# itmo153277/JoshUpscale

Hardware: AMD Instinct MI355X
Metric: frames/sec 480x270->1920x1080 recurrent SR (higher is better)
Workload: dtype bf16

## Files before the change

### joshupscale_amd/csrc/dev_switch.cpp

```cpp
#include "dev_switch.h"

#ifdef JU_TEST_HOOKS
#include <cstdlib>
#endif

namespace ju {

#ifdef JU_TEST_HOOKS
const char *devSwitch(Dev which) {
	static const char *const kNames[static_cast<int>(Dev::Count)] = {
	    "JU_TAIL", "JU_PACK", "JU_POOL", "JU_UPSAMPLE", "JU_FLOW_CONV", "JU_TOWER", "JU_CALIBRATE", "JU_FLOW", "JU_DIRECT",
	    "JU_DIRECT_GRAPH", "JU_SYNC_SPIN_US", "JU_TRACE_STEPS", "JU_TRACE_NOSYNC", "JU_RES_BLOCK", "JU_FLOW_TILE",
	    "JU_FLOW_WIDE", "JU_WAVE_PRIO", "JU_CONV_DBUF", "JU_TOWER_FAST", "JU_FP8_GRID", "JU_FP8_BLOCK",
	};
	const int i = static_cast<int>(which);
	if (i < 0 || i >= static_cast<int>(Dev::Count)) return nullptr;
	return std::getenv(kNames[i]);
}
#else
const char *devSwitch(Dev) {
	return nullptr;
}
#endif

}
```

### joshupscale_amd/csrc/dev_switch.h

```cpp
#pragma once

namespace ju {

enum class Dev : int {
	Tail,
	Pack,
	Pool,
	Upsample,
	FlowConv,
	Tower,
	Calibrate,
	Flow,
	Direct,
	DirectGraph,
	SyncSpinUs,
	TraceSteps,
	TraceNoSync,
	ResBlock,
	FlowTile,
	FlowWide,
	WavePrio,
	ConvDbuf,
	TowerFast,
	Fp8Grid,
	Fp8Block,
	Count
};

const char *devSwitch(Dev which);

}
```

### joshupscale_amd/csrc/engine.cpp

```cpp
#include "engine.h"

#include <cstdio>

#include <algorithm>
#include <atomic>
#include <cstdlib>
#include <cstring>
#include <memory>
#include <mutex>
#include <sstream>
#include <stdexcept>

#include "dev_switch.h"
#include "fp8.h"
#include "graphics.h"
#include "log.h"

namespace ju {

namespace {
thread_local int g_DryLaunches = 0;
}
bool launchesAreDry() { return g_DryLaunches > 0; }
DryLaunchScope::DryLaunchScope() { ++g_DryLaunches; }
// ... 284 lines not shown
	const int PH = c.paddedHeight(), PW = c.paddedWidth();
	const int padTop = (PH - H) / 2, padLeft = (PW - W) / 2;
	const FrameIO *io = &m_IO;
	const FrameIO *batchIO = m_BatchIO;
	const void *const *groupPrev = m_GroupPrev;
	void *const *groupOut = m_GroupOut;
	const void *packedIn = m_Packed[set].get();
	void *packedOut = m_Packed[set ^ 1].get();
	const int nIn = c.numFlowInputs;
	const unsigned *sums = c.normalizeBrightness ? m_TailB2.as<unsigned>() + 4 : nullptr;
	auto T = [&](const std::string &n) -> void * { return (batch ? m_BatchTensors : m_Tensors).at(n).buf.get(); };
	auto Op = [&](const std::string &n) { return batch ? Operand{T(n), 0} : operand(n); };
	auto itemBytes = [&](const std::string &n) -> long {
		const Tensor &t = m_Tensors.at(n);
		return static_cast<long>(t.count) * (t.isF32 ? 4 : 2);
	};
	auto noBatch = [&](const char *what) {
		if (batch) throw std::logic_error(std::string("look-ahead: no batched form of ") + what);
	};
	const Operand none{};
	const bool packInBlock = flowPacksInBlock();
	if (batch && (!packInBlock || sums != nullptr)) noBatch("the input packing");
	Operand cur{packedOut, 0};
	long curItem = 0;
	int h = PH, w = PW;
	bool flowHeadDone = false;
	const int nb = static_cast<int>(c.flowFilters.size()) / 2;
	auto fusesUpsample = [&](const std::string &next, int cin) {
		auto it = m_Convs.find(next);
		return m_FusedUpsample && it != m_Convs.end() && cin % 64 == 0 && it->second.nb == 1 &&
		       it->second.cout <= 32;
	};
	const int flowAct = c.flowActivation == 1 ? 2 : 1;
	auto addBlockStep = [&](const std::string &convA, const std::string &convB, const void *in, long inItem,
	                        const std::string &outName, int bh, int bw, bool ups, bool pool, bool outHead, int act2) {
		const ConvWeights &wa = m_Convs.at(convA), &wb = m_Convs.at(convB);
		FlowBlockLaunch fb{};
		fb.in = in;
		fb.w1 = wa.w.get();
		fb.b1 = wa.bias.as<float>();
		fb.w2 = wb.w.get();
		fb.b2 = wb.bias.as<float>();
		fb.out = T(outName);
		fb.H = bh;
		fb.W = bw;
		fb.cin = wa.cinP;
		fb.cmid = wa.cout;
		fb.upsample = ups;
		fb.pool = pool;
		fb.outHead = outHead;
		fb.act1 = flowAct;
		fb.act2 = act2;
		fb.slope = c.flowNegativeSlope;
		fb.items = items;
		fb.inItemBytes = inItem;
		fb.outItemBytes = itemBytes(outName);
		const double flops =
		    items * 2.0 * bh * bw * 9.0 * (double(wa.cinReal) * wa.cout + double(wb.cinReal) * wb.cout);
		if (packInBlock && convA == "flow/block_1/conv_1") {
			fb.packPrev = packedIn;
			fb.packOut = packedOut;
			fb.frameH = H;
			fb.frameW = W;
			fb.padTop = padTop;
			fb.padLeft = padLeft;
			fb.numInputs = nIn;
			fb.sums = sums;
			if (group) {
				fb.packPrev = nullptr;
				fb.packOut = nullptr;
				fb.independentItems = true;
			}
			prog.push_back({"flow", flops, [dt, fb, io, batchIO, groupPrev, groupOut, items, group](hipStream_t s) {
				                FlowBlockLaunch f = fb;
				                f.packFrame = io->in;
				                f.packFrameStride = io->inStride;
				                for (int i = 0; i < items && (items > 1 || group); ++i) {
					                f.packFrames[i] = batchIO[i].in;
					                f.packFrameStrides[i] = batchIO[i].inStride;
					                if (group) {
						                f.packPrevs[i] = groupPrev[i];
						                f.packOuts[i] = groupOut[i];
					                }
				                }
				                launchFlowBlock(dt, f, s);
			                }});
			return;
		}
		prog.push_back({"flow", flops, [dt, fb](hipStream_t s) { launchFlowBlock(dt, fb, s); }});
	};
	auto unitUpsIn = [&](int k) { return k < static_cast<int>(m_FlowUnits.size()) && m_FlowUnits[k].fused && m_FlowUnits[k].upsIn; };
	bool upsampleNext = false;
	for (int i = 0; i < 2 * nb; ++i) {
		const std::string n = "flow/block_" + std::to_string(i + 1);
		const int f = c.flowFilters[i];
		if (m_FlowUnits[i].fused) {
			const bool pool = i < nb;
			if (upsampleNext != m_FlowUnits[i].upsIn) throw std::logic_error("flow plan out of step");
			addBlockStep(n + "/conv_1", n + "/conv_2", cur.ptr, curItem, pool ? n + "/resample" : n + "/a_2", h, w,
			    upsampleNext, pool, false, flowAct);
			upsampleNext = false;
			if (pool) {
				h /= 2;
				w /= 2;
				cur = Operand{T(n + "/resample"), 0};
				curItem = itemBytes(n + "/resample");
// ... 100 lines not shown
	const FrameIO *io = &m_IO;
	const void *packedIn = m_Packed[set].get();
	void *packedOut = m_Packed[set ^ 1].get();
	m_StateBind[set].in = m_State[c.recurrent() ? set : 0].get();
	m_StateBind[set].out = m_State[c.recurrent() ? set ^ 1 : 0].get();
	const StateBind *sb = &m_StateBind[set];
	const int nIn = c.numFlowInputs;
	auto T = [&](const std::string &n) -> void * { return m_Tensors.at(n).buf.get(); };
	auto Op = [&](const std::string &n) { return operand(n); };
	const Operand none{};

	const unsigned *sums = c.normalizeBrightness && c.recurrent() ? m_TailB2.as<unsigned>() + 4 : nullptr;
	std::uint8_t *const discard = c.outputsPreWarp() ? m_DiscardFrame.as<std::uint8_t>() : nullptr;
	const std::ptrdiff_t discardStride = static_cast<std::ptrdiff_t>(W) * 16;
	auto genOutU8 = [=] { return discard ? discard : io->out; };
	auto genOutStride = [=] { return discard ? discardStride : io->outStride; };
	if (!c.recurrent()) {
		const Operand genInOp = Op("gen_in");
		void *genIn = genInOp.ptr;
		const int genPitch = genInOp.pitch;
		prog.push_back({"lr_pack", 0.0,
		    [=](hipStream_t s) { launchLrPack(dt, io->in, io->inStride, genIn, genPitch, H, W, s); }});
	}
	if (sums) {
		unsigned *sumsOut = m_TailB2.as<unsigned>() + 4;
		prog.push_back({"pack", 0.0,
		    [=](hipStream_t s) { launchFrameSums(io->in, io->inStride, H, W, sumsOut, s); }});
	}
	const bool packInBlock = flowPacksInBlock();
	if (!packInBlock && c.recurrent()) {
		prog.push_back({"pack", 0.0, [=](hipStream_t s) {
			                launchPackFrames(dt, io->in, io->inStride, packedIn, packedOut, H, W, PH, PW,
			                    padTop, padLeft, nIn, sums, s);
		                }});
	}
	auto addResBlockStep = [&](const std::string &tag, const std::string &block, Operand in, Operand out,
	                           int bh, int bw, int act, float slope) {
		const ConvWeights &wa = m_Convs.at(block + "/conv_1"), &wb = m_Convs.at(block + "/conv_2");
		FlowBlockLaunch fb{};
		fb.in = in.ptr;
		fb.inPitch = in.pitch;
		fb.w1 = wa.wBlock.get();
		fb.b1 = wa.bias.as<float>();
		fb.w2 = wb.wBlock.get();
		fb.b2 = wb.bias.as<float>();
		fb.out = out.ptr;
		fb.outPitch = out.pitch;
		fb.H = bh;
		fb.W = bw;
		fb.cin = fb.cmid = 64;
		fb.residual = true;
		fb.act1 = fb.act2 = act;
		fb.slope = slope;
		prog.push_back({tag, 2.0 * bh * bw * 9.0 * 64 * 64 * 2,
		    [dt, fb](hipStream_t s) { launchFlowBlock(dt, fb, s); }});
	};
	Operand cur{packedOut, 0};
	int h = PH, w = PW;
	bool flowHeadDone = false;
	if (!c.recurrent()) {
		flowHeadDone = true;
	} else if (c.flowArch == 0) {
		addFlowAutoencoder(&prog, set, 1);
		flowHeadDone = true;
	} else if (m_ResidentFlow) {
		void *in64 = T("flow/in64");
		prog.push_back({"flow", 0.0,
		    [=](hipStream_t s) { launchExpandChannels(dt, packedOut, in64, PH * PW, s); }});
		ResidentTowerParams rp{};
		rp.in = in64;
		rp.inPitch = PW;
		rp.hasHead = 1;
		rp.out = Op("flow/trunk").ptr;
		rp.weights = m_FlowTowerW.get();
		rp.bias = m_FlowTowerB.as<float>();
		rp.mailbox = m_FlowMail.get();
		rp.counters = m_FlowFlags.as<unsigned>();
		rp.error = m_ResErrorDev;
		rp.debug = m_Tensors.at("tower_profile").buf.get();
		rp.H = PH;
		rp.W = PW;
		rp.GX = m_FlowGX;
		rp.GY = m_FlowGY;
		rp.RH = m_FlowRH;
		rp.nLayers = 1 + 2 * c.flowResBlocks;
		rp.leaky = c.flowActivation == 1 ? 1 : 0;
		rp.slope = c.flowNegativeSlope;
		prog.push_back({"flow",
		    2.0 * PH * PW * 9.0 * (3.0 * c.numFlowInputs * 64 + 64.0 * 64 * 2 * c.flowResBlocks),
		    [=](hipStream_t s) { launchResidentTower(dt, rp, s); }});
		cur = Op("flow/trunk");
	} else {
		addConvStep(&prog, "flow", "flow/conv_1", cur, none, Op("flow/x0"), h, w, true, false);
		const char *xs[2] = {"flow/x0", "flow/x1"};
		int a = 0;
		for (int i = 0; i < c.flowResBlocks; ++i) {
			const std::string n = "flow/block_" + std::to_string(i + 1);
			if (m_BlockFused && c.flowResFilters == 64) {
				addResBlockStep("flow", n, Op(xs[a]), Op(xs[a ^ 1]), h, w, c.flowActivation == 1 ? 2 : 1,
				    c.flowNegativeSlope);
				a ^= 1;
				continue;
			}
			addConvStep(&prog, "flow", n + "/conv_1", Op(xs[a]), none, Op("flow/t"), h, w, true, false);
			addConvStep(&prog, "flow", n + "/conv_2", Op("flow/t"), Op(xs[a]), Op(xs[a ^ 1]), h, w,
			    true, false);
// ... 237 lines not shown
			                launchTail(dt, y, w2, b2, io->in, io->inStride, sb->out, genOutU8(),
			                    genOutStride(), H, W, sums, s);
		                }});
	}
	if (c.temporalStrength > 0.0f) {
		const void *preWarp = T("pre_warp");
		unsigned long long *acc = m_TemporalAcc.as<unsigned long long>();
		const TemporalParams tp{c.temporalStrength, c.temporalThreshold, c.temporalGain, c.temporalWindow,
		    c.temporalL2 ? 1 : 0, c.temporalLimit ? 1 : 0, c.temporalLuma ? 1 : 0};
		prog.push_back({"temporal", 0.0, [=](hipStream_t s) {
			                launchTemporalFilter(sb->out, preWarp, genOutU8(), genOutStride(), H, W, sums,
			                    acc, tp, s);
		                }});
	}
}

Engine::Engine(int device, const void *blob, std::size_t size, int dtypeOverride)
    : m_Device(device) {
	int current = -1;
	JU_HIP(hipGetDevice(&current));
	if (current != device) throw std::logic_error("Engine must be created with its device current");
	ModelFile model(blob, size);
	m_Config = model.config();
	const ModelConfig &c = m_Config;
	int dt = dtypeOverride >= 0 ? dtypeOverride : c.computeDtype;
	m_ModelDigest = 14695981039346656037ull;
	for (std::size_t i = 0; i < size; ++i) {
		m_ModelDigest = (m_ModelDigest ^ static_cast<const unsigned char *>(blob)[i]) * 1099511628211ull;
	}
	m_DtypeOverride = dt;
	if (dt == 2) {
		if (c.genFilters != 64 || c.genBlocks < 1) {
			throw std::invalid_argument("fp8 tower needs a 64-filter generator with at least one residual block");
		}
		m_Fp8Tower = true;
		dt = kF16;
	}
	if (dt != kF16 && dt != kBF16) throw std::invalid_argument("Unsupported compute dtype");
	m_DType = static_cast<DType>(dt);
	const int H = c.frameHeight, W = c.frameWidth;
	const int PH = c.paddedHeight(), PW = c.paddedWidth();

	const char *tailMode = devSwitch(Dev::Tail);
	m_FusedTail = !(tailMode && std::string(tailMode) == "split");
	m_TailInTower = !(tailMode && (std::string(tailMode) == "fused" || std::string(tailMode) == "split"));
	const char *packMode = devSwitch(Dev::Pack);
	m_PackInBlock = !(packMode && std::string(packMode) == "split");
	const char *poolMode = devSwitch(Dev::Pool);
	m_FusedPool = !(poolMode && std::string(poolMode) == "split");
	const char *upMode = devSwitch(Dev::Upsample);
	m_FusedUpsample = !(upMode && std::string(upMode) == "split");
	const char *flowConv = devSwitch(Dev::FlowConv);
	m_FlowFused = !(flowConv && std::string(flowConv) == "generic") && m_FusedUpsample;
	planFlowUnits();

	buildWeights(model);

	{
		const char *mode = devSwitch(Dev::Tower);
		int cus = 0;
		JU_HIP(hipDeviceGetAttribute(&cus, hipDeviceAttributeMultiprocessorCount, device));
		bool wanted = !(mode && (std::string(mode) == "layers" || std::string(mode) == "convs"));
		m_BlockFused = !(mode && std::string(mode) == "convs");
		const char *calib = devSwitch(Dev::Calibrate);
		m_Calibrate = calib && calib[0] == '1';
		if (m_Calibrate) {
			if (m_Fp8Tower) throw std::invalid_argument("calibration mode: calibrate the fp16 / bf16 engine, not the 8-bit one");
			wanted = false;
			m_BlockFused = false;
		}
		if (wanted && c.genFilters == 64 && c.genBlocks >= 1 &&
		    residentTowerGeometry(c.frameHeight, c.frameWidth, cus, &m_ResGX, &m_ResGY, &m_ResRH)) {
			m_Resident = m_ResidentCapable = true;
			m_TowerW = DeviceBuffer(m_TowerHostW.size() * 2);
			m_TowerW.upload(m_TowerHostW.data(), m_TowerHostW.size() * 2);
			m_TowerB = DeviceBuffer(m_TowerHostB.size() * 4);
			m_TowerB.upload(m_TowerHostB.data(), m_TowerHostB.size() * 4);
			m_ResMail = DeviceBuffer(m_Fp8Tower ? residentMailboxBytes8(m_ResGX, m_ResGY, c.genActivation == 1)
			                                    : residentMailboxBytes(m_ResGX, m_ResGY, c.genActivation == 1));
			m_ResFlags = DeviceBuffer(residentCounterBytes(m_ResGX, m_ResGY));
			m_ResError = PinnedWords(64);
			m_ResErrorDev = m_ResError.device();
		}
		m_TowerHostW.clear();
		m_TowerHostW.shrink_to_fit();
		const char *flowMode = devSwitch(Dev::Flow);
		if (flowMode && std::string(flowMode) == "convs") m_BlockFused = false;
		if (m_Resident && !(flowMode && (std::string(flowMode) == "layers" || std::string(flowMode) == "convs")) &&
		    c.flowArch == 1 &&
		    c.flowResFilters == 64 && c.flowResBlocks >= 1 && 3 * c.numFlowInputs <= 64 &&
		    residentTowerGeometry(PH, PW, cus, &m_FlowGX, &m_FlowGY, &m_FlowRH)) {
			m_ResidentFlow = m_ResidentFlowCapable = true;
			m_FlowTowerW = DeviceBuffer(m_FlowTowerHostW.size() * 2);
			m_FlowTowerW.upload(m_FlowTowerHostW.data(), m_FlowTowerHostW.size() * 2);
			m_FlowTowerB = DeviceBuffer(m_FlowTowerHostB.size() * 4);
			m_FlowTowerB.upload(m_FlowTowerHostB.data(), m_FlowTowerHostB.size() * 4);
			m_FlowMail = DeviceBuffer(residentMailboxBytes(m_FlowGX, m_FlowGY, c.flowActivation == 1));
			m_FlowFlags = DeviceBuffer(residentCounterBytes(m_FlowGX, m_FlowGY));
		}
		m_FlowTowerHostW.clear();
		m_FlowTowerHostW.shrink_to_fit();
	}

	const std::size_t lr = static_cast<std::size_t>(H) * W;
	const std::size_t plr = static_cast<std::size_t>(PH) * PW;
	m_InStage = DeviceBuffer(lr * 4);
// ... 1698 lines not shown
```

### joshupscale_amd/csrc/engine.h

```cpp
#pragma once

#include <cstddef>
#include <cstdint>
#include <functional>
#include <map>
#include <memory>
#include <mutex>
#include <set>
#include <string>
#include <tuple>
#include <vector>

#include "hip_util.h"
#include "kernels.h"
#include "model.h"

namespace ju {

enum class Location : std::uint8_t { Host = 0, Device = 1, GraphicsResource = 2 };

struct Frame {
	void *ptr;
	Location location;
	std::ptrdiff_t stride;
// ... 120 lines not shown
	void runProgram();
	struct FrameIO {
		const std::uint8_t *in = nullptr;
		std::ptrdiff_t inStride = 0;
		std::uint8_t *out = nullptr;
		std::ptrdiff_t outStride = 0;
	};
	FrameIO m_IO;
	struct StateBind {
		const void *in = nullptr;
		void *out = nullptr;
	};
	StateBind m_StateBind[2];
	const void *m_FlowCur = nullptr;
	bool m_DirectIO = false;
	bool m_PreferDirect = true;
	void submit(const Frame &in, const Frame &out);

	int m_Device;
	ModelConfig m_Config;
	DType m_DType;
	Stream m_Stream;
	bool m_UseGraph = true;
	unsigned m_SpinUs = 2000;
	int m_Idx = 0;
	std::string m_TrunkOut = "trunk_a";

	std::map<std::string, Tensor> m_Tensors;
	std::map<std::string, ConvWeights> m_Convs;
	struct Fp8Conv {
		DeviceBuffer w, scaleA;
	};
	bool m_Fp8Tower = false;
	std::map<std::string, Fp8Conv> m_Fp8Convs;
	std::map<std::string, FoldedConv> m_Fp8Folded;
	DeviceBuffer m_Fp8X, m_Fp8T;
	std::vector<int> m_Fp8Exp;
	DeviceBuffer m_Fp8TowerW, m_Fp8TowerScaleA, m_Fp8TowerBias, m_Fp8TowerScaleB, m_Fp8TowerMul;
	DeviceBuffer m_TailW2, m_TailB2, m_TailW2Frag;
	DeviceBuffer m_Zeros;
	DeviceBuffer m_TemporalAcc;
	struct FlowUnit {
		bool fused = false;
		bool upsIn = false;
	};
	std::vector<FlowUnit> m_FlowUnits;
	bool m_FlowFused = true;
	bool m_BlockFused = true;
	bool m_Calibrate = false;
	void planFlowUnits();
	bool flowConvIsFused(const std::string &name) const;
	bool m_FusedUpsample = true;
	bool m_FusedPool = true;
	bool m_PackInBlock = true;
	bool m_FusedTail = true;
	bool m_TailInTower = false;
	DeviceBuffer m_InStage, m_OutStage, m_RawStage;
	DeviceBuffer m_DiscardFrame;
	DeviceBuffer m_State[2], m_Packed[2];
	bool m_Resident = false;
	int m_ResGX = 0, m_ResGY = 0, m_ResRH = 0;
	std::vector<std::uint16_t> m_TowerHostW;
	std::vector<float> m_TowerHostB;
	DeviceBuffer m_TowerW, m_TowerB, m_ResMail, m_ResFlags;
	bool m_ResidentFlow = false;
	int m_FlowGX = 0, m_FlowGY = 0, m_FlowRH = 0;
	std::vector<std::uint16_t> m_FlowTowerHostW;
	std::vector<float> m_FlowTowerHostB;
	DeviceBuffer m_FlowTowerW, m_FlowTowerB, m_FlowMail, m_FlowFlags;
	bool m_ResidentCapable = false, m_ResidentFlowCapable = false;
	unsigned m_RetryBase = 512, m_RetryAfter = 0, m_CleanFrames = 0, m_Fallbacks = 0;
	void restoreResident();
	void maybeRestoreResident();
	Event m_FrameDone;
	std::unique_lock<std::mutex> chainBegin();
	void chainEnd(std::unique_lock<std::mutex> &lock);
	PinnedWords m_ResError;
	unsigned *m_ResErrorDev = nullptr;
	unsigned takeResidentError();
	void fallbackToLayers(unsigned code);
	std::vector<Step> m_Program[2];
	GraphExec m_Graph[2];
	struct DirectKey {
		const void *in;
		std::ptrdiff_t inStride;
		void *out;
		std::ptrdiff_t outStride;
		int idx;
		bool operator<(const DirectKey &o) const {
			return std::tie(in, inStride, out, outStride, idx) <
			       std::tie(o.in, o.inStride, o.out, o.outStride, o.idx);
		}
	};
	struct DirectEntry {
		GraphExec graph;
		unsigned seen = 0;
		std::uint64_t lastUse = 0;
		bool registered = false;
	};
	std::map<DirectKey, DirectEntry> m_DirectGraphs;
	std::set<DirectKey> m_RegisteredPairs;
	bool directEligible(const Frame &in, const Frame &out) const;
	DirectEntry &directEntry(const DirectKey &key);
	void captureDirect(DirectEntry *e, int idx);
	FrameIO m_BatchIO[kFlowBatchMax];
	struct YuvKey {
// ... 73 lines not shown
```

### joshupscale_amd/csrc/flow_kernels.hip

```cpp
#include "flow_block_common.h"

namespace ju {

namespace {

struct FlowBlockParams {
	const void *in;
	const void *w1;
	const float *b1;
	const void *w2;
	const float *b2;
	void *out;
	int H, W;
	int inPitch, outPitch;
	int act1, act2;
	float slope;
	int skip;
	int prio;
	const void *packPrev;
	void *packOut;
	int frameH, frameW, padTop, padLeft, numInputs;
	const unsigned *sums;
	long inItem, outItem;
	const std::uint8_t *frames[kFlowBatchMax];
	std::ptrdiff_t frameStrides[kFlowBatchMax];
	const void *packPrevs[kFlowBatchMax];
	void *packOuts[kFlowBatchMax];
};

template <int CIN, int CMID, int TH, bool UPS, bool POOL, int OUTK, int NW = 4>
struct FbGeom {
	static constexpr int CK1 = CIN >= 64 ? 64 : CIN;
	static constexpr int NPL = CIN / CK1;
	static constexpr int PBX = CK1 * 2;
	static constexpr int KS1 = CK1 / 16;
	static constexpr int XR = TH + 4;
	static constexpr int TR = TH + 2;
	static constexpr int XPLANE = XR * kFbW * PBX;
	static constexpr int PBT = CMID * 2;
	static constexpr int KS2 = CMID / 16;
	static constexpr int NCB = CMID / 32;
	static constexpr int TBYTES = TR * kFbW * PBT;
	static constexpr int LR = XR / 2 + 1, LC = kFbW / 2 + 1;
	static constexpr int LBYTES = UPS ? NPL * LR * LC * PBX : 0;
	static constexpr bool XPAIR = UPS && NPL > 2 && TH > 2;
	static constexpr int NPLX = XPAIR ? 2 : NPL;
	static constexpr int OFF_X = 0;
	static constexpr int OFF_T = NPLX * XPLANE;
	static constexpr int TREGION = TBYTES > LBYTES ? TBYTES : LBYTES;
	static constexpr int ESZ = 2;
	static constexpr int RBW = 32 * ESZ;
	static constexpr int STAGE_PX = POOL ? 16 : 64;
	static constexpr int STAGE_WAVE = STAGE_PX * RBW;
	static constexpr bool STAGE_IN_X = NPLX * XPLANE >= NW * STAGE_WAVE;
	static constexpr int OFF_STAGE = STAGE_IN_X ? OFF_X : OFF_T + TREGION;
	static constexpr int LDS = OFF_T + TREGION + (STAGE_IN_X ? 0 : NW * STAGE_WAVE);
	static_assert(CIN == 16 || CIN == 32 || CIN == 64 || CIN == 128 || CIN == 256, "input channels");
#ifndef JU_FB_RELOAD_MIN
#define JU_FB_RELOAD_MIN 3
#endif
	static constexpr bool RELOAD = NPL >= JU_FB_RELOAD_MIN;
	static_assert(CMID == 32 || CMID == 64 || CMID == 128, "block filters");
	static_assert(NW % NCB == 0, "cout blocks over the waves");
	static_assert(TH % 2 == 0 && TH >= 2, "row pairs");
	static constexpr bool FITS = LDS <= 160 * 1024;
};

template <typename T, int CIN, int CMID, int TH, bool UPS, bool POOL, int OUTK, int NW, bool PACK = false, bool INDEP = false>
__global__ __launch_bounds__(NW * 64, NW / 4) void flow_block_kernel(FlowBlockParams p) {
	static_assert(!PACK || (CIN == 16 && !UPS), "PACK: the 16-channel flow input");
	static_assert(!INDEP || PACK, "INDEP: a form of the input packing");
	using G = FbGeom<CIN, CMID, TH, UPS, POOL, OUTK, NW>;
	constexpr int NT = NW * 64;
	extern __shared__ __attribute__((aligned(16))) unsigned char smem[];
	const int tid = threadIdx.x;
	const int wave = tid >> 6;
	if constexpr (NW == 8) applyWavePriority(p.prio, wave, NW);
	const int lane = tid & 63;
	const int px = lane & 31;
	const int hh = lane >> 5;
	const int x0 = blockIdx.x * kFbOutW;
	const int y0 = blockIdx.y * TH;
	const int item = blockIdx.z;
	const T *__restrict__ in = reinterpret_cast<const T *>(static_cast<const unsigned char *>(p.in) + item * p.inItem);
	const unsigned ldsBase = static_cast<unsigned>(reinterpret_cast<unsigned long long>(
	    (__attribute__((address_space(3))) unsigned char *)smem));

	constexpr int NCB = G::NCB;
	const int cb = wave % NCB;
	const int pstart = wave / NCB;
	constexpr int PSTEP = NW / NCB;
	const float s1 = fbActS(p.act1, p.slope), s2 = fbActS(p.act2, p.slope);

	constexpr int NWA = G::RELOAD ? ((NW == 4 && !G::XPAIR) ? 2 : 1) : G::NPL;
	Vec8<T> wa[NWA][9 * G::KS1];
	const unsigned char *waSrc = static_cast<const unsigned char *>(p.w1) +
	                             (size_t)cb * G::NPL * (9 * G::KS1 * 1024) + lane * 16;
	auto loadPlaneA = [&](int set, int pl) __attribute__((always_inline)) {
#pragma unroll
		for (int f = 0; f < 9 * G::KS1; ++f) {
			wa[set][f] = *reinterpret_cast<const Vec8<T> *>(waSrc + (size_t)(pl * 9 * G::KS1 + f) * 1024);
		}
	};
	if constexpr (G::RELOAD) {
		loadPlaneA(0, 0);
	} else {
#pragma unroll
		for (int pl = 0; pl < G::NPL; ++pl) loadPlaneA(pl, pl);
	}

	[[maybe_unused]] constexpr int LPPX = G::PBX / 16;
	[[maybe_unused]] auto expandPlanes = [&](int plFirst, int plCount) __attribute__((always_inline)) {
		if constexpr (UPS) {
			constexpr int LPP = LPPX;
			constexpr int NPIX = G::LR * G::LC;
			const unsigned char *smL = smem + G::OFF_T;
			constexpr int BR = G::XR / 2, BC = kFbW / 2;
			const int nel = plCount * BR * BC * LPP;
			for (int e = tid; e < nel; e += NT) {
				const int c = e % LPP;
				const int bq = (e / LPP) % (BR * BC);
				const int pl = plFirst + e / (LPP * BR * BC);
				const int br = bq / BC, bc = bq - br * BC;
				const unsigned char *base = smL + pl * (NPIX * G::PBX) + (br * G::LC + bc) * G::PBX + c * 16;
				const Vec8<T> tl = *reinterpret_cast<const Vec8<T> *>(base);
				const Vec8<T> tr = *reinterpret_cast<const Vec8<T> *>(base + G::PBX);
				const Vec8<T> bl = *reinterpret_cast<const Vec8<T> *>(base + G::LC * G::PBX);
				const Vec8<T> brr = *reinterpret_cast<const Vec8<T> *>(base + (G::LC + 1) * G::PBX);
				Vec8<T> o01, o10, o11;
#pragma unroll
				for (int j = 0; j < 8; ++j) {
					const float a = static_cast<float>(tl[j]), b2 = static_cast<float>(tr[j]);
					const float d = static_cast<float>(bl[j]), e2 = static_cast<float>(brr[j]);
					const float top = a + (b2 - a) * 0.5f;
					const float bot = d + (e2 - d) * 0.5f;
					o01[j] = static_cast<T>(top);
					o10[j] = static_cast<T>(a + (d - a) * 0.5f);
					o11[j] = static_cast<T>(top + (bot - top) * 0.5f);
				}
				const int r = 2 * br, k = 2 * bc;
				const int gy = y0 - 2 + r, gx = x0 - 2 + k;
				const Vec8<T> zero = {static_cast<T>(0.f), static_cast<T>(0.f), static_cast<T>(0.f), static_cast<T>(0.f),
				    static_cast<T>(0.f), static_cast<T>(0.f), static_cast<T>(0.f), static_cast<T>(0.f)};
				const bool inside = gy >= 0 && gy < p.H && gx >= 0 && gx < p.W;
				unsigned char *xb = smem + G::OFF_X + (G::XPAIR ? (pl & 1) : pl) * G::XPLANE + (r * kFbW + k) * G::PBX;
				const unsigned s0 = (static_cast<unsigned>(c) ^ fbSwz<G::PBX>(k)) << 4;
				const unsigned s1x = (static_cast<unsigned>(c) ^ fbSwz<G::PBX>(k + 1)) << 4;
				*reinterpret_cast<Vec8<T> *>(xb + s0) = inside ? tl : zero;
				*reinterpret_cast<Vec8<T> *>(xb + G::PBX + s1x) = inside ? o01 : zero;
				*reinterpret_cast<Vec8<T> *>(xb + kFbW * G::PBX + s0) = inside ? o10 : zero;
				*reinterpret_cast<Vec8<T> *>(xb + (kFbW + 1) * G::PBX + s1x) = inside ? o11 : zero;
			}
		}
	};
	const bool border = y0 - 2 < 0 || y0 + TH + 2 > p.H || x0 - 2 < 0 || x0 + 32 > p.W;
	constexpr int LPP = G::PBX / 16;
	if (JU_SKIP(p) & 1) {
	} else if constexpr (PACK) {
		const float bright = brightnessOf(p.sums, 1.0f / static_cast<float>(p.frameH * p.frameW));
		const T *__restrict__ prev = static_cast<const T *>(INDEP ? p.packPrevs[item] : p.packPrev);
		T *__restrict__ cur = INDEP ? static_cast<T *>(p.packOuts[item])
		                            : (item + 1 == static_cast<int>(gridDim.z) ? static_cast<T *>(p.packOut) : nullptr);
		const int nch = 3 * p.numInputs;
		const int fromFrames = INDEP ? 1 : min(item + 1, p.numInputs);
		constexpr int NPIX = G::XR * kFbW;
		for (int q = tid; q < NPIX; q += NT) {
			const int r = q / kFbW, k = q - r * kFbW;
			const int gy = y0 - 2 + r, gx = x0 - 2 + k;
			const T zero = static_cast<T>(0.f);
			Vec8<T> o0 = {zero, zero, zero, zero, zero, zero, zero, zero}, o1 = o0;
			const bool inside = gy >= 0 && gy < p.H && gx >= 0 && gx < p.W;
			if (inside) {
				const int y = gy - p.padTop, x = gx - p.padLeft;
				const bool inFrame = y >= 0 && y < p.frameH && x >= 0 && x < p.frameW;
				const size_t idx = (size_t)gy * p.W + gx;
				T pv[16], o[16];
#pragma unroll
				for (int j = 0; j < 16; ++j) o[j] = zero;
#pragma unroll
				for (int h = 0; h < 5; ++h) {
					if (h < fromFrames) {
						float c0 = 0.f, c1 = 0.f, c2 = 0.f;
						if (inFrame) {
							const unsigned v = *reinterpret_cast<const unsigned *>(p.frames[item - h] + y * p.frameStrides[item - h] + x * 4);
							c0 = preprocessU8(v & 0xff) - bright;
							c1 = preprocessU8((v >> 8) & 0xff) - bright;
							c2 = preprocessU8((v >> 16) & 0xff) - bright;
						}
						o[3 * h] = static_cast<T>(c0);
						o[3 * h + 1] = static_cast<T>(c1);
						o[3 * h + 2] = static_cast<T>(c2);
					}
				}
				if (fromFrames < p.numInputs) {
					const Vec8<T> p0 = *reinterpret_cast<const Vec8<T> *>(prev + idx * 16);
					const Vec8<T> p1 = *reinterpret_cast<const Vec8<T> *>(prev + idx * 16 + 8);
#pragma unroll
					for (int i = 0; i < 8; ++i) {
						pv[i] = p0[i];
						pv[8 + i] = p1[i];
					}
					auto shifted = [&](auto sTag) __attribute__((always_inline)) {
						constexpr int S = decltype(sTag)::value;
#pragma unroll
						for (int j = S; j < 16; ++j) o[j] = (j < nch) ? pv[j - S] : zero;
					};
					if (fromFrames == 1) shifted(std::integral_constant<int, 3>{});
					else if (fromFrames == 2) shifted(std::integral_constant<int, 6>{});
					else if (fromFrames == 3) shifted(std::integral_constant<int, 9>{});
					else shifted(std::integral_constant<int, 12>{});
				}
#pragma unroll
				for (int i = 0; i < 8; ++i) {
					o0[i] = o[i];
					o1[i] = o[8 + i];
				}
				if (cur != nullptr && r >= 2 && r < 2 + TH && k >= 2 && k < 2 + kFbOutW) {
					*reinterpret_cast<Vec8<T> *>(cur + idx * 16) = o0;
					*reinterpret_cast<Vec8<T> *>(cur + idx * 16 + 8) = o1;
				}
			}
			unsigned char *xb = smem + G::OFF_X + (r * kFbW + k) * G::PBX;
			const unsigned sw = fbSwz<G::PBX>(k);
			*reinterpret_cast<Vec8<T> *>(xb + ((0u ^ sw) << 4)) = o0;
			*reinterpret_cast<Vec8<T> *>(xb + ((1u ^ sw) << 4)) = o1;
		}
		__syncthreads();
	} else if constexpr (!UPS) {
		if (border) {
			for (int i = tid; i < G::NPL * G::XPLANE / 16; i += NT) {
				reinterpret_cast<uint4 *>(smem + G::OFF_X)[i] = make_uint4(0, 0, 0, 0);
			}
			__syncthreads();
		}
		constexpr int NPXI = 1024 / G::PBX;
		constexpr int NPIX = G::XR * kFbW;
		constexpr int NINSTR = (NPIX + NPXI - 1) / NPXI;
#pragma unroll
		for (int pl = 0; pl < G::NPL; ++pl) {
			for (int i = wave; i < NINSTR; i += NW) {
				const int q = i * NPXI + lane / LPP;
				const int r = q / kFbW, k = q - r * kFbW;
				const int gy = y0 - 2 + r, gx = x0 - 2 + k;
				const unsigned c = static_cast<unsigned>(lane % LPP) ^ fbSwz<G::PBX>(k);
				if (q < NPIX && gy >= 0 && gy < p.H && gx >= 0 && gx < p.W) {
					fbGlds16(in + ((size_t)gy * p.inPitch + gx) * CIN + pl * 64 + c * 8,
					    smem + G::OFF_X + pl * G::XPLANE + i * 1024);
				}
			}
		}
		asm volatile("s_waitcnt vmcnt(0)" ::: "memory");
		__syncthreads();
	} else {
		unsigned char *smL = smem + G::OFF_T;
		const int lh = p.H >> 1, lw = p.W >> 1;
		const int ly0 = (y0 >> 1) - 1, lx0 = (x0 >> 1) - 1;
		constexpr int NPXI = 1024 / G::PBX;
		constexpr int NPIX = G::LR * G::LC;
		constexpr int NINSTR = (NPIX + NPXI - 1) / NPXI;
#pragma unroll
		for (int pl = 0; pl < G::NPL; ++pl) {
			for (int i = wave; i < NINSTR; i += NW) {
				const int q = min(i * NPXI + lane / LPP, NPIX - 1);
				const int r = q / G::LC, k = q - r * G::LC;
				const int cy = min(max(ly0 + r, 0), lh - 1), cx = min(max(lx0 + k, 0), lw - 1);
				if (i * NPXI + lane / LPP < NPIX) {
					fbGlds16(in + ((size_t)cy * p.inPitch + cx) * CIN + pl * 64 + (lane % LPP) * 8,
					    smL + pl * (NPIX * G::PBX) + i * 1024);
				}
			}
		}
		asm volatile("s_waitcnt vmcnt(0)" ::: "memory");
		__syncthreads();
		if constexpr (!G::XPAIR) {
			expandPlanes(0, G::NPL);
		} else {
			expandPlanes(0, 1);
		}
		__syncthreads();
	}

	unsigned colOffA[3], colSwzA[3];
#pragma unroll
	for (int dx = 0; dx < 3; ++dx) {
		colOffA[dx] = (px + dx) * G::PBX;
		colSwzA[dx] = fbSwz<G::PBX>(px + dx);
	}
	{
		constexpr int NPAIR = G::TR / 2;
		constexpr int MAXP = (NPAIR + PSTEP - 1) / PSTEP;
		constexpr int HOLD = G::NPL > 1 ? MAXP : 1;
		f32x16 acc[HOLD][2];
		unsigned tOff[4];
#pragma unroll
		for (int g = 0; g < 4; ++g) {
			tOff[g] = px * G::PBT + ((static_cast<unsigned>(cb * 4 + g) ^ fbSwz<G::PBT>(px)) << 4) + hh * 8;
		}
		constexpr bool kHoistBiasA = NWA * 9 * G::KS1 * 4 < 144 || NW == 4;
		f32x4 biasA[4];
		if constexpr (kHoistBiasA) {
#pragma unroll
			for (int g = 0; g < 4; ++g) biasA[g] = *reinterpret_cast<const f32x4 *>(p.b1 + cb * 32 + 8 * g + 4 * hh);
		}
		auto initAcc = [&](f32x16(&a)[2]) {
#pragma unroll
			for (int g = 0; g < 4; ++g) {
				f32x4 bg;
				if constexpr (kHoistBiasA) bg = biasA[g];
				else bg = *reinterpret_cast<const f32x4 *>(p.b1 + cb * 32 + 8 * g + 4 * hh);
#pragma unroll
				for (int r = 0; r < 2; ++r) {
#pragma unroll
					for (int i = 0; i < 4; ++i) a[r][4 * g + i] = bg[i];
				}
			}
		};
		auto epilogueA = [&](const f32x16(&a)[2], int pair) {
			const int gx = x0 - 1 + px;
			const bool colIn = gx >= 0 && gx < p.W;
#pragma unroll
			for (int r = 0; r < 2; ++r) {
				const int tr = 2 * pair + r;
				const int gy = y0 - 1 + tr;
				const float keep = (colIn && gy >= 0 && gy < p.H) ? 1.0f : 0.0f;
				unsigned char *row = smem + G::OFF_T + tr * (kFbW * G::PBT);
#pragma unroll
				for (int g = 0; g < 4; ++g) {
					*reinterpret_cast<Vec4<T> *>(row + tOff[g]) =
					    pack4<T>(fbAct(a[r][4 * g + 0], s1) * keep, fbAct(a[r][4 * g + 1], s1) * keep,
					        fbAct(a[r][4 * g + 2], s1) * keep, fbAct(a[r][4 * g + 3], s1) * keep);
				}
			}
		};
		if (JU_SKIP(p) & 2) {
		} else if constexpr (G::NPL == 1) {
			for (int pair = pstart; pair < NPAIR; pair += PSTEP) {
				initAcc(acc[0]);
				FbPair<T, G::KS1, G::PBX>::run(ldsBase + G::OFF_X + (2 * pair) * (kFbW * G::PBX), colOffA, colSwzA,
				    hh, wa[0], acc[0]);
				epilogueA(acc[0], pair);
			}
		} else {
#pragma unroll
			for (int s = 0; s < HOLD; ++s) initAcc(acc[s]);
#pragma unroll
			for (int pl = 0; pl < G::NPL; ++pl) {
				if constexpr (G::RELOAD && NWA == 2) {
					if (pl + 1 < G::NPL) loadPlaneA((pl + 1) & 1, pl + 1);
				}
				if constexpr (G::XPAIR) {
					if (pl + 1 < G::NPL && !(JU_SKIP(p) & 1)) expandPlanes(pl + 1, 1);
				}
#pragma unroll
				for (int s = 0; s < HOLD; ++s) {
					const int pair = pstart + s * PSTEP;
					if (pair < NPAIR) {
						FbPair<T, G::KS1, G::PBX>::run(
						    ldsBase + G::OFF_X + (G::XPAIR ? (pl & 1) : pl) * G::XPLANE + (2 * pair) * (kFbW * G::PBX), colOffA,
						    colSwzA, hh, wa[G::RELOAD ? (pl & (NWA - 1)) : pl], acc[s]);
					}
				}
				if constexpr (G::RELOAD && NWA == 1) {
					if (pl + 1 < G::NPL) loadPlaneA(0, pl + 1);
				}
				if constexpr (G::XPAIR) __syncthreads();
			}
#pragma unroll
			for (int s = 0; s < HOLD; ++s) {
				const int pair = pstart + s * PSTEP;
				if (pair < NPAIR) epilogueA(acc[s], pair);
			}
		}
	}

	Vec8<T> wb[9 * G::KS2];
	f32x4 biasB[4];
	{
		const unsigned char *wsrc = static_cast<const unsigned char *>(p.w2) + (size_t)cb * (9 * G::KS2 * 1024) + lane * 16;
#pragma unroll
		for (int f = 0; f < 9 * G::KS2; ++f) {
			constexpr int KSP = G::KS2 > 4 ? 4 : G::KS2;
			const int tap = f / G::KS2, ks = f % G::KS2;
			wb[f] = *reinterpret_cast<const Vec8<T> *>(wsrc + (size_t)(((ks / KSP) * 9 + tap) * KSP + ks % KSP) * 1024);
		}
#pragma unroll
		for (int g = 0; g < 4; ++g) biasB[g] = *reinterpret_cast<const f32x4 *>(p.b2 + cb * 32 + 8 * g + 4 * hh);
	}
	__syncthreads();

	unsigned colOffB[3], colSwzB[3];
#pragma unroll
	for (int dx = 0; dx < 3; ++dx) {
		colOffB[dx] = (px + dx) * G::PBT;
		colSwzB[dx] = fbSwz<G::PBT>(px + dx);
	}
	unsigned char *stage = smem + G::OFF_STAGE + wave * G::STAGE_WAVE;
	constexpr int NCH = G::RBW / 16;
	for (int pair = pstart; pair < ((JU_SKIP(p) & 4) ? 0 : TH / 2); pair += PSTEP) {
		f32x16 acc[2];
#pragma unroll
		for (int g = 0; g < 4; ++g) {
#pragma unroll
			for (int r = 0; r < 2; ++r) {
#pragma unroll
				for (int i = 0; i < 4; ++i) acc[r][4 * g + i] = biasB[g][i];
			}
		}
		FbPair<T, G::KS2, G::PBT>::run(ldsBase + G::OFF_T + (2 * pair) * (kFbW * G::PBT), colOffB, colSwzB, hh, wb, acc);
		Vec4<T> resv[2][4];
		if constexpr (OUTK == 2) {
			static_assert(CIN == CMID && !UPS && !POOL, "residual block: same width in and out");
#pragma unroll
			for (int r = 0; r < 2; ++r) {
				const int gy = min(y0 + 2 * pair + r, p.H - 1), gx = min(x0 + px, p.W - 1);
				const T *rp = in + ((size_t)gy * p.inPitch + gx) * CIN + cb * 32 + 4 * hh;
#pragma unroll
				for (int g = 0; g < 4; ++g) resv[r][g] = *reinterpret_cast<const Vec4<T> *>(rp + 8 * g);
			}
		}
		if constexpr (POOL) {
			const int pp = px >> 1;
#pragma unroll
			for (int g = 0; g < 4; ++g) {
				float v[4];
#pragma unroll
				for (int i = 0; i < 4; ++i) {
					float m = fmaxf(acc[0][4 * g + i], acc[1][4 * g + i]);
					m = fmaxf(m, fbSwapPair(m));
					v[i] = fbAct(m, s2);
				}
				if ((g >> 1) == (px & 1)) {
					const unsigned c = static_cast<unsigned>(g) ^ (static_cast<unsigned>(pp) & (NCH - 1));
					*reinterpret_cast<Vec4<T> *>(stage + pp * G::RBW + (c << 4) + hh * 8) = pack4<T>(v[0], v[1], v[2], v[3]);
				}
			}
		} else {
// ... 91 lines not shown
	long bestCost = 0;
	auto consider = [&](int TH, bool fits) {
		if (!fits) return;
		const long c = fbForcedTile() == TH ? -1 : fbLaunchCost(p.H, tilesX, TH, numCUs, items);
		if (best == 0 || c < bestCost) {
			best = TH;
			bestCost = c;
		}
	};
	(consider(THS, FbGeom<CIN, CMID, THS, UPS, POOL, OUTK, fbWaves<CIN, CMID>()>::FITS), ...);
	bool done = false;
	auto launch = [&](auto thTag) {
		constexpr int TH = decltype(thTag)::value;
		if constexpr (FbGeom<CIN, CMID, TH, UPS, POOL, OUTK, fbWaves<CIN, CMID>()>::FITS) {
			if (!done && best == TH) {
				launchFlowBlockInst<T, CIN, CMID, TH, UPS, POOL, OUTK, PACK, INDEP>(p, items, stream);
				done = true;
			}
		}
	};
	(launch(std::integral_constant<int, THS>{}), ...);
	if (!done) throw std::logic_error("flow block: no tile height fits");
}

template <typename T, int CIN, int CMID, bool UPS, bool POOL, int OUTK, bool PACK = false, bool INDEP = false>
void launchFlowBlockT(const FlowBlockParams &p, int items, int numCUs, hipStream_t stream) {
	if constexpr (OUTK == 2) {
		launchFlowBlockBest<T, CIN, CMID, UPS, POOL, OUTK, PACK, INDEP, kFbMid, 6>(p, items, numCUs, stream);
	} else if constexpr (CMID == 128) {
		launchFlowBlockBest<T, CIN, CMID, UPS, POOL, OUTK, PACK, INDEP, 6, 4, 2>(p, items, numCUs, stream);
	} else {
		launchFlowBlockBest<T, CIN, CMID, UPS, POOL, OUTK, PACK, INDEP, 20, 18, 10, 6>(p, items, numCUs, stream);
	}
}

template <typename T>
void launchFlowBlockDT(const FlowBlockLaunch &q, hipStream_t stream) {
	FlowBlockParams p{};
	p.in = q.in;
	p.w1 = q.w1;
	p.b1 = q.b1;
	p.w2 = q.w2;
	p.b2 = q.b2;
	p.out = q.out;
	p.H = q.H;
	p.W = q.W;
	p.inPitch = q.inPitch ? q.inPitch : (q.upsample ? q.W / 2 : q.W);
	p.outPitch = q.outPitch ? q.outPitch : (q.pool ? q.W / 2 : q.W);
	p.act1 = q.act1;
	p.act2 = q.act2;
	p.slope = q.slope;
	p.skip = ablationSkipBits();
	p.prio = wavePriorityMode(0);
	p.packPrev = q.packPrev;
	p.packOut = q.packOut;
	p.frameH = q.frameH;
	p.frameW = q.frameW;
	p.padTop = q.padTop;
	p.padLeft = q.padLeft;
	p.numInputs = q.numInputs;
	p.sums = q.sums;
	const int items = q.items > 1 ? q.items : 1;
	if (items > kFlowBatchMax) throw std::invalid_argument("flow block: more look-ahead frames than kFlowBatchMax");
	p.inItem = items > 1 ? q.inItemBytes : 0;
	p.outItem = items > 1 ? q.outItemBytes : 0;
	const bool many = items > 1 || q.independentItems;
	for (int i = 0; i < kFlowBatchMax; ++i) {
		p.frames[i] = many ? (i < items ? q.packFrames[i] : nullptr) : (i == 0 ? q.packFrame : nullptr);
		p.frameStrides[i] = many ? (i < items ? q.packFrameStrides[i] : 0) : (i == 0 ? q.packFrameStride : 0);
		p.packPrevs[i] = q.independentItems && i < items ? q.packPrevs[i] : nullptr;
		p.packOuts[i] = q.independentItems && i < items ? q.packOuts[i] : nullptr;
	}
	if (items > 1 && q.residual) throw std::invalid_argument("flow block: the residual form has no look-ahead launch");
	const int cus = currentDeviceCUs();
	if (q.packOut != nullptr || q.independentItems) {
		if (many && q.sums != nullptr) throw std::invalid_argument("flow block: look-ahead packing has no brightness sums");
		for (int i = 0; i < items; ++i) {
			if (p.frames[i] == nullptr) throw std::invalid_argument("flow block: input packing needs every frame of the launch");
			if (q.independentItems && (p.packPrevs[i] == nullptr || p.packOuts[i] == nullptr)) {
				throw std::invalid_argument("flow block: independent items need every item's history buffers");
			}
		}
		if (!(q.cin == 16 && q.cmid == 32 && !q.upsample && q.pool && !q.outHead && !q.residual &&
		        (q.packPrev || q.independentItems))) {
			throw std::invalid_argument("flow block: input packing is built for the first block (16 -> 32 -> 32, pool)");
		}
		if (q.independentItems) return launchFlowBlockT<T, 16, 32, false, true, 0, true, true>(p, items, cus, stream);
		return launchFlowBlockT<T, 16, 32, false, true, 0, true>(p, items, cus, stream);
	}
	if (q.upsample && (q.H % 2 || q.W % 2)) throw std::invalid_argument("flow block: fused upsampling needs even H and W");
	if (q.pool && (q.H % 2 || q.W % 2)) throw std::invalid_argument("flow block: fused max-pool needs even H and W");
	const int outk = q.residual ? 2 : (q.outHead ? 1 : 0);
#define JU_FB_CASE(CIN_, CMID_, UPS_, POOL_, OUTK_)                                              \
	if (q.cin == CIN_ && q.cmid == CMID_ && q.upsample == UPS_ && q.pool == POOL_ && outk == OUTK_) { \
		return launchFlowBlockT<T, CIN_, CMID_, UPS_, POOL_, OUTK_>(p, items, cus, stream);         \
	}
	JU_FB_CASE(16, 32, false, true, 0)
	JU_FB_CASE(32, 64, false, true, 0)
	JU_FB_CASE(64, 128, false, true, 0)
	JU_FB_CASE(256, 128, true, false, 0)
	JU_FB_CASE(256, 128, false, false, 0)
	JU_FB_CASE(128, 64, true, false, 0)
	JU_FB_CASE(128, 64, false, false, 0)
	JU_FB_CASE(64, 32, true, false, 1)
	JU_FB_CASE(64, 32, false, false, 1)
	JU_FB_CASE(64, 64, false, false, 2)
// ... 39 lines not shown
```

### joshupscale_amd/csrc/kernels.h

```cpp
#pragma once

#include <hip/hip_runtime_api.h>

#include <cstddef>
#include <cstdint>

namespace ju {

enum DType : int { kF16 = 0, kBF16 = 1 };

inline std::size_t dtypeSize(DType) { return 2; }

struct ConvParams {
	const void *in;
	const void *wgt;
	const float *bias;
	const void *res;
	void *out;
	int H, W;
	int cin, cout;
	int taps;
	int relu;
	float slope;
	int outHead;
// ... 17 lines not shown

constexpr long kConvTargetWgs = 512;
inline void convTiling(int H, int W, int cout, int *nb, int *rw) {
	const int tilesX = (W + 31) / 32;
	int bestNb = 1, bestRw = 1;
	long bestWgs = -1;
	const int nbs[2] = {2, 1};
	const int rws[2] = {2, 1};
	for (int a = 0; a < 2; ++a) {
		if (cout % (32 * nbs[a]) != 0) continue;
		for (int b = 0; b < 2; ++b) {
			const long wgs = (long)tilesX * ((H + 4 * rws[b] - 1) / (4 * rws[b])) * (cout / (32 * nbs[a]));
			if (wgs >= ((a == 0 && b == 0) ? 256 : kConvTargetWgs)) {
				*nb = nbs[a];
				*rw = rws[b];
				return;
			}
			if (wgs > bestWgs) {
				bestWgs = wgs;
				bestNb = nbs[a];
				bestRw = rws[b];
			}
		}
	}
	*nb = bestNb;
	*rw = bestRw;
}

void launchConv(DType dt, const ConvParams &p, hipStream_t stream);

bool launchesAreDry();
struct DryLaunchScope {
	DryLaunchScope();
	~DryLaunchScope();
	DryLaunchScope(const DryLaunchScope &) = delete;
	DryLaunchScope &operator=(const DryLaunchScope &) = delete;
};

constexpr int kFlowBatchMax = 8;
struct FlowBlockLaunch {
	const void *in;
	const void *w1;
	const float *b1;
	const void *w2;
	const float *b2;
	void *out;
	int H, W;
	int inPitch, outPitch;
	int cin, cmid;
	bool upsample, pool, outHead;
	bool residual;
	int act1, act2;
	float slope;
	const std::uint8_t *packFrame;
	std::ptrdiff_t packFrameStride;
	const void *packPrev;
	void *packOut;
	int frameH, frameW, padTop, padLeft, numInputs;
	const unsigned *sums;
	int items;
	long inItemBytes, outItemBytes;
	const std::uint8_t *packFrames[kFlowBatchMax];
	std::ptrdiff_t packFrameStrides[kFlowBatchMax];
	bool independentItems;
	const void *packPrevs[kFlowBatchMax];
	void *packOuts[kFlowBatchMax];
};
bool flowBlockSupported(int cin, int cmid, bool upsample, bool pool, bool outHead, int H = 0, int W = 0);
void launchFlowBlock(DType dt, const FlowBlockLaunch &q, hipStream_t stream);

bool convSplitKSupported(const ConvParams &p);
void launchConvSplitK(DType dt, const ConvParams &p, const void *zeros, hipStream_t stream);

void launchConvTower(DType dt, const ConvParams &p, hipStream_t stream);

struct Fp8TowerParams {
	const void *in8;
	const void *weights;
	const int *scaleA;
	const float *bias;
	void *stream;
	void *out8;
	int inExp;
	int outExp;
	int H, W;
	int leaky;
	float slope;
};
void launchConvTowerFp8(DType dt, const Fp8TowerParams &p, hipStream_t stream);
struct Fp8BlockLaunch {
	const void *in8;
	void *out8;
	void *stream;
	const void *w1, *w2;
	const int *scaleA1, *scaleA2;
	const float *b1, *b2;
	int inExp, midExp, outExp;
	int H, W;
	int leaky;
	float slope;
};
void launchResBlockFp8(DType dt, const Fp8BlockLaunch &q, hipStream_t stream);
void launchQuantizeTower(DType dt, const void *in, void *out8, int H, int W, int exponent, bool leaky,
    hipStream_t stream);

struct ResidentTowerParams {
// ... 172 lines not shown
```

Before: 2168.

## Stage flow-block conv weights in LDS and prefetch conv B weights early

```diff
diff --git a/joshupscale_amd/csrc/dev_switch.cpp b/joshupscale_amd/csrc/dev_switch.cpp
--- a/joshupscale_amd/csrc/dev_switch.cpp
+++ b/joshupscale_amd/csrc/dev_switch.cpp
@@ -12,6 +12,7 @@
 	    "JU_TAIL", "JU_PACK", "JU_POOL", "JU_UPSAMPLE", "JU_FLOW_CONV", "JU_TOWER", "JU_CALIBRATE", "JU_FLOW", "JU_DIRECT",
 	    "JU_DIRECT_GRAPH", "JU_SYNC_SPIN_US", "JU_TRACE_STEPS", "JU_TRACE_NOSYNC", "JU_RES_BLOCK", "JU_FLOW_TILE",
 	    "JU_FLOW_WIDE", "JU_WAVE_PRIO", "JU_CONV_DBUF", "JU_TOWER_FAST", "JU_FP8_GRID", "JU_FP8_BLOCK",
+	    "JU_FB_WEIGHTS",
 	};
 	const int i = static_cast<int>(which);
 	if (i < 0 || i >= static_cast<int>(Dev::Count)) return nullptr;
diff --git a/joshupscale_amd/csrc/dev_switch.h b/joshupscale_amd/csrc/dev_switch.h
--- a/joshupscale_amd/csrc/dev_switch.h
+++ b/joshupscale_amd/csrc/dev_switch.h
@@ -24,6 +24,7 @@
 	TowerFast,
 	Fp8Grid,
 	Fp8Block,
+	FlowWeights,
 	Count
 };
 
diff --git a/joshupscale_amd/csrc/engine.cpp b/joshupscale_amd/csrc/engine.cpp
--- a/joshupscale_amd/csrc/engine.cpp
+++ b/joshupscale_amd/csrc/engine.cpp
@@ -360,6 +360,7 @@
 		fb.act1 = flowAct;
 		fb.act2 = act2;
 		fb.slope = c.flowNegativeSlope;
+		fb.privateWeights = m_FlowWeightsPrivate;
 		fb.items = items;
 		fb.inItemBytes = inItem;
 		fb.outItemBytes = itemBytes(outName);
@@ -566,6 +567,7 @@
 		fb.residual = true;
 		fb.act1 = fb.act2 = act;
 		fb.slope = slope;
+		fb.privateWeights = m_FlowWeightsPrivate;
 		prog.push_back({tag, 2.0 * bh * bw * 9.0 * 64 * 64 * 2,
 		    [dt, fb](hipStream_t s) { launchFlowBlock(dt, fb, s); }});
 	};
@@ -909,6 +911,8 @@
 	m_FusedUpsample = !(upMode && std::string(upMode) == "split");
 	const char *flowConv = devSwitch(Dev::FlowConv);
 	m_FlowFused = !(flowConv && std::string(flowConv) == "generic") && m_FusedUpsample;
+	const char *fbWeights = devSwitch(Dev::FlowWeights);
+	m_FlowWeightsPrivate = fbWeights && std::string(fbWeights) == "private";
 	planFlowUnits();
 
 	buildWeights(model);
diff --git a/joshupscale_amd/csrc/engine.h b/joshupscale_amd/csrc/engine.h
--- a/joshupscale_amd/csrc/engine.h
+++ b/joshupscale_amd/csrc/engine.h
@@ -196,6 +196,7 @@
 	bool flowConvIsFused(const std::string &name) const;
 	bool m_FusedUpsample = true;
 	bool m_FusedPool = true;
+	bool m_FlowWeightsPrivate = false;
 	bool m_PackInBlock = true;
 	bool m_FusedTail = true;
 	bool m_TailInTower = false;
diff --git a/joshupscale_amd/csrc/flow_kernels.hip b/joshupscale_amd/csrc/flow_kernels.hip
--- a/joshupscale_amd/csrc/flow_kernels.hip
+++ b/joshupscale_amd/csrc/flow_kernels.hip
@@ -17,6 +17,7 @@
 	float slope;
 	int skip;
 	int prio;
+	int wpriv;
 	const void *packPrev;
 	void *packOut;
 	int frameH, frameW, padTop, padLeft, numInputs;
@@ -54,17 +55,29 @@
 	static constexpr int STAGE_WAVE = STAGE_PX * RBW;
 	static constexpr bool STAGE_IN_X = NPLX * XPLANE >= NW * STAGE_WAVE;
 	static constexpr int OFF_STAGE = STAGE_IN_X ? OFF_X : OFF_T + TREGION;
-	static constexpr int LDS = OFF_T + TREGION + (STAGE_IN_X ? 0 : NW * STAGE_WAVE);
+	static constexpr int LDS0 = OFF_T + TREGION + (STAGE_IN_X ? 0 : NW * STAGE_WAVE);
 	static_assert(CIN == 16 || CIN == 32 || CIN == 64 || CIN == 128 || CIN == 256, "input channels");
 #ifndef JU_FB_RELOAD_MIN
 #define JU_FB_RELOAD_MIN 3
 #endif
 	static constexpr bool RELOAD = NPL >= JU_FB_RELOAD_MIN;
+	static constexpr int WBBYTES = NCB * 9 * KS2 * 1024;
+	static constexpr int WABYTES = NCB * NPL * 9 * KS1 * 1024;
+	static constexpr bool WB_LDS = NW == 8 && NW > NCB && LDS0 + WBBYTES <= 160 * 1024;
+	static constexpr bool WA_LDS = WB_LDS && !RELOAD && LDS0 + WBBYTES + WABYTES <= 160 * 1024;
+	static constexpr int OFF_WB = LDS0;
+	static constexpr int OFF_WA = LDS0 + WBBYTES;
+	static constexpr int LDS = LDS0 + (WB_LDS ? WBBYTES : 0) + (WA_LDS ? WABYTES : 0);
 	static_assert(CMID == 32 || CMID == 64 || CMID == 128, "block filters");
 	static_assert(NW % NCB == 0, "cout blocks over the waves");
 	static_assert(TH % 2 == 0 && TH >= 2, "row pairs");
-	static constexpr bool FITS = LDS <= 160 * 1024;
+	static constexpr bool FITS = LDS0 <= 160 * 1024;
+	static_assert(!FITS || LDS <= 160 * 1024, "weight areas only where they fit");
 };
+static_assert(FbGeom<16, 32, 18, false, true, 0, 8>::WA_LDS && FbGeom<16, 32, 18, false, true, 0, 8>::LDS <= 96 * 1024, "block 1: both sets");
+static_assert(FbGeom<32, 64, 6, false, true, 0, 8>::WB_LDS && !FbGeom<32, 64, 6, false, true, 0, 8>::WA_LDS, "block 2: conv B's");
+static_assert(FbGeom<64, 32, 18, true, false, 1, 8>::WB_LDS && !FbGeom<64, 32, 18, true, false, 1, 8>::WA_LDS, "head: conv B's");
+static_assert(!FbGeom<128, 64, 6, true, false, 0, 4>::WB_LDS && !FbGeom<64, 128, 2, false, true, 0, 4>::WB_LDS, "4 waves: per wave");
 
 template <typename T, int CIN, int CMID, int TH, bool UPS, bool POOL, int OUTK, int NW, bool PACK = false, bool INDEP = false>
 __global__ __launch_bounds__(NW * 64, NW / 4) void flow_block_kernel(FlowBlockParams p) {
@@ -102,12 +115,47 @@
 			wa[set][f] = *reinterpret_cast<const Vec8<T> *>(waSrc + (size_t)(pl * 9 * G::KS1 + f) * 1024);
 		}
 	};
+	const bool shared = p.wpriv == 0;
 	if constexpr (G::RELOAD) {
 		loadPlaneA(0, 0);
-	} else {
+	} else if (!(G::WA_LDS && shared)) {
 #pragma unroll
 		for (int pl = 0; pl < G::NPL; ++pl) loadPlaneA(pl, pl);
 	}
+	if constexpr (G::WB_LDS) {
+		if (shared) {
+			const unsigned char *src = static_cast<const unsigned char *>(p.w2) + lane * 16;
+			for (int i = wave; i < G::WBBYTES / 1024; i += NW) fbGlds16(src + (size_t)i * 1024, smem + G::OFF_WB + i * 1024);
+			if constexpr (G::WA_LDS) {
+				const unsigned char *srcA = static_cast<const unsigned char *>(p.w1) + lane * 16;
+				for (int i = wave; i < G::WABYTES / 1024; i += NW) fbGlds16(srcA + (size_t)i * 1024, smem + G::OFF_WA + i * 1024);
+			}
+		}
+	}
+	constexpr int NFB = 9 * G::KS2;
+	Vec8<T> wb[NFB];
+	auto srcIndexB = [](int f) __attribute__((always_inline)) {
+		constexpr int KSP = G::KS2 > 4 ? 4 : G::KS2;
+		const int tap = f / G::KS2, ks = f % G::KS2;
+		return ((ks / KSP) * 9 + tap) * KSP + ks % KSP;
+	};
+	const unsigned char *wbSrc = static_cast<const unsigned char *>(p.w2) + (size_t)cb * (NFB * 1024) + lane * 16;
+	auto loadB = [&](int f0, int f1) __attribute__((always_inline)) {
+#pragma unroll
+		for (int f = 0; f < NFB; ++f) {
+			if (f >= f0 && f < f1) wb[f] = *reinterpret_cast<const Vec8<T> *>(wbSrc + (size_t)srcIndexB(f) * 1024);
+		}
+	};
+	constexpr bool kEarlyB = !G::WB_LDS && NW == 4 && !G::XPAIR && (G::NPL > 1 || 9 * G::KS1 < 92);
+	constexpr int kFragBudget = 92 - 9 * G::KS1;
+	constexpr bool kHoistBiasA = NWA * 9 * G::KS1 * 4 < 144 || NW == 4;
+	constexpr bool kBiasAFirst = kHoistBiasA && kEarlyB && G::NPL == 1;
+	f32x4 biasA[4];
+	if constexpr (kBiasAFirst) {
+#pragma unroll
+		for (int g = 0; g < 4; ++g) biasA[g] = *reinterpret_cast<const f32x4 *>(p.b1 + cb * 32 + 8 * g + 4 * hh);
+	}
+	constexpr int NEARLY = !kEarlyB ? 0 : (G::NPL == 1 ? (NFB < kFragBudget ? NFB : kFragBudget) : (NFB < 9 * G::KS1 ? NFB : 9 * G::KS1));
 
 	[[maybe_unused]] constexpr int LPPX = G::PBX / 16;
 	[[maybe_unused]] auto expandPlanes = [&](int plFirst, int plCount) __attribute__((always_inline)) {
@@ -156,6 +204,10 @@
 	const bool border = y0 - 2 < 0 || y0 + TH + 2 > p.H || x0 - 2 < 0 || x0 + 32 > p.W;
 	constexpr int LPP = G::PBX / 16;
 	if (JU_SKIP(p) & 1) {
+		if constexpr (G::WB_LDS) {
+			asm volatile("s_waitcnt vmcnt(0)" ::: "memory");
+			__syncthreads();
+		}
 	} else if constexpr (PACK) {
 		const float bright = brightnessOf(p.sums, 1.0f / static_cast<float>(p.frameH * p.frameW));
 		const T *__restrict__ prev = static_cast<const T *>(INDEP ? p.packPrevs[item] : p.packPrev);
@@ -225,6 +277,7 @@
 			*reinterpret_cast<Vec8<T> *>(xb + ((0u ^ sw) << 4)) = o0;
 			*reinterpret_cast<Vec8<T> *>(xb + ((1u ^ sw) << 4)) = o1;
 		}
+		if constexpr (G::WB_LDS) asm volatile("s_waitcnt vmcnt(0)" ::: "memory");
 		__syncthreads();
 	} else if constexpr (!UPS) {
 		if (border) {
@@ -280,6 +333,22 @@
 		__syncthreads();
 	}
 
+	if constexpr (G::WA_LDS) {
+		if (shared) {
+#pragma unroll
+			for (int pl = 0; pl < G::NPL; ++pl) {
+#pragma unroll
+				for (int f = 0; f < 9 * G::KS1; ++f) {
+					wa[pl][f] = *reinterpret_cast<const Vec8<T> *>(
+					    smem + G::OFF_WA + ((cb * G::NPL + pl) * 9 * G::KS1 + f) * 1024 + lane * 16);
+				}
+			}
+		}
+	}
+	if constexpr (kEarlyB && G::NPL == 1) {
+		if (shared) loadB(0, NEARLY);
+	}
+
 	unsigned colOffA[3], colSwzA[3];
 #pragma unroll
 	for (int dx = 0; dx < 3; ++dx) {
@@ -296,9 +365,7 @@
 		for (int g = 0; g < 4; ++g) {
 			tOff[g] = px * G::PBT + ((static_cast<unsigned>(cb * 4 + g) ^ fbSwz<G::PBT>(px)) << 4) + hh * 8;
 		}
-		constexpr bool kHoistBiasA = NWA * 9 * G::KS1 * 4 < 144 || NW == 4;
-		f32x4 biasA[4];
-		if constexpr (kHoistBiasA) {
+		if constexpr (kHoistBiasA && !kBiasAFirst) {
 #pragma unroll
 			for (int g = 0; g < 4; ++g) biasA[g] = *reinterpret_cast<const f32x4 *>(p.b1 + cb * 32 + 8 * g + 4 * hh);
 		}
@@ -348,6 +415,9 @@
 				if constexpr (G::RELOAD && NWA == 2) {
 					if (pl + 1 < G::NPL) loadPlaneA((pl + 1) & 1, pl + 1);
 				}
+				if constexpr (kEarlyB && G::NPL > 1) {
+					if (pl + 1 == G::NPL && shared) loadB(0, NEARLY);
+				}
 				if constexpr (G::XPAIR) {
 					if (pl + 1 < G::NPL && !(JU_SKIP(p) & 1)) expandPlanes(pl + 1, 1);
 				}
@@ -373,15 +443,22 @@
 		}
 	}
 
-	Vec8<T> wb[9 * G::KS2];
 	f32x4 biasB[4];
 	{
-		const unsigned char *wsrc = static_cast<const unsigned char *>(p.w2) + (size_t)cb * (9 * G::KS2 * 1024) + lane * 16;
-#pragma unroll
-		for (int f = 0; f < 9 * G::KS2; ++f) {
-			constexpr int KSP = G::KS2 > 4 ? 4 : G::KS2;
-			const int tap = f / G::KS2, ks = f % G::KS2;
-			wb[f] = *reinterpret_cast<const Vec8<T> *>(wsrc + (size_t)(((ks / KSP) * 9 + tap) * KSP + ks % KSP) * 1024);
+		if constexpr (G::WB_LDS) {
+			if (shared) {
+#pragma unroll
+				for (int f = 0; f < NFB; ++f) {
+					wb[f] = *reinterpret_cast<const Vec8<T> *>(smem + G::OFF_WB + (cb * NFB + srcIndexB(f)) * 1024 + lane * 16);
+				}
+			} else {
+				loadB(0, NFB);
+			}
+		} else if constexpr (NEARLY > 0) {
+			if (shared) loadB(NEARLY, NFB);
+			else loadB(0, NFB);
+		} else {
+			loadB(0, NFB);
 		}
 #pragma unroll
 		for (int g = 0; g < 4; ++g) biasB[g] = *reinterpret_cast<const f32x4 *>(p.b2 + cb * 32 + 8 * g + 4 * hh);
@@ -579,6 +656,7 @@
 	p.slope = q.slope;
 	p.skip = ablationSkipBits();
 	p.prio = wavePriorityMode(0);
+	p.wpriv = q.privateWeights ? 1 : 0;
 	p.packPrev = q.packPrev;
 	p.packOut = q.packOut;
 	p.frameH = q.frameH;
diff --git a/joshupscale_amd/csrc/kernels.h b/joshupscale_amd/csrc/kernels.h
--- a/joshupscale_amd/csrc/kernels.h
+++ b/joshupscale_amd/csrc/kernels.h
@@ -93,6 +93,7 @@
 	bool residual;
 	int act1, act2;
 	float slope;
+	bool privateWeights;
 	const std::uint8_t *packFrame;
 	std::ptrdiff_t packFrameStride;
 	const void *packPrev;
```

After: 2163. No clear change (-0.2%).
